# sahaRatul/sela

Hardware: NVIDIA H100
Metric: encode+decode MSamples/s (higher is better)
Workload: dtype f64+int64

## Files before the change

sela_b200/csrc/c_abi.cu:

```cuda
#include <algorithm>
#include <atomic>
#include <cstdarg>
#include <cstdio>
#include <cstdlib>
#include <cstring>
#include <mutex>
#include <thread>
#include <vector>

#include "verify.cuh"

using namespace selab200;

namespace {

thread_local char g_error[512] = "";
std::mutex g_mutex;
std::atomic<uint64_t> g_launches{0};

int fail(int code, const char *fmt, ...)
{
    va_list ap;
    va_start(ap, fmt);
    vsnprintf(g_error, sizeof g_error, fmt, ap);
// ... 180 lines not shown
    if (g_n_ctx == 0)
        return require_ready();
    cudaPointerAttributes attr;
    if (cudaPointerGetAttributes(&attr, device_ptr) != cudaSuccess || attr.type != cudaMemoryTypeDevice) {
        cudaGetLastError();
        return fail(SELAB200_ERR_ARGUMENT, "not a device pointer");
    }
    for (int i = 0; i < g_n_ctx; i++)
        if (g_slots[i].ready && g_slots[i].device == attr.device) {
            tl_ctx = &g_slots[i];
            cudaError_t e = cudaSetDevice(g.device);
            if (e != cudaSuccess)
                return fail(SELAB200_ERR_CUDA, "cudaSetDevice(%d) failed: %s", g.device, cudaGetErrorString(e));
            return 0;
        }
    return fail(SELAB200_ERR_ARGUMENT, "the buffers live on device %d, which the library was not initialised for "
                                       "(selab200_init / selab200_init_devices)", attr.device);
}

size_t align256(size_t v) { return (v + 255) & ~(size_t)255; }

template <typename K>
int set_smem(K kernel, size_t bytes)
{
    static std::mutex m;
    static std::vector<std::pair<std::pair<const void *, int>, size_t>> done;
    int dev = 0;
    CUDA_TRY(cudaGetDevice(&dev));
    const std::pair<const void *, int> key(reinterpret_cast<const void *>(kernel), dev);
    std::lock_guard<std::mutex> lock(m);
    for (auto &e : done)
        if (e.first == key) {
            if (e.second >= bytes)
                return 0;
            CUDA_TRY(cudaFuncSetAttribute(kernel, cudaFuncAttributeMaxDynamicSharedMemorySize, (int)bytes));
            e.second = bytes;
            return 0;
        }
    CUDA_TRY(cudaFuncSetAttribute(kernel, cudaFuncAttributeMaxDynamicSharedMemorySize, (int)bytes));
    done.emplace_back(key, bytes);
    return 0;
}

int launch_check(const char *what)
{
    g_launches.fetch_add(1, std::memory_order_relaxed);
    cudaError_t e = cudaGetLastError();
    if (e != cudaSuccess)
        return fail(SELAB200_ERR_CUDA, "launch of %s failed: %s", what, cudaGetErrorString(e));
    return 0;
}

template <int KIND>
int launch_unit_means(const void *src, size_t n_units, uint32_t channels, double *means, cudaStream_t stream)
{
    const MeanTiling mt = mean_tiling(KIND, channels);
    k_unit_means<KIND><<<(unsigned)((n_units + 31) / 32), 32, unit_means_smem_bytes(mt), stream>>>(src, (uint32_t)n_units,
                                                                                                 channels, means);
    return launch_check("k_unit_means");
}

template <bool STEREO, bool TRACE>
int launch_encode_units(const EncodeParams &p, size_t n_units, selab200_analysis_trace *d_trace, cudaStream_t stream)
{
    constexpr size_t smem = encode_smem_bytes<STEREO>();
    if (int rc = set_smem(k_encode_units<STEREO, TRACE>, smem))
        return rc;
    k_encode_units<STEREO, TRACE><<<(unsigned)n_units, 32, smem, stream>>>(p, d_trace);
    return launch_check("k_encode_units");
}


int encode_device(const int16_t *d_pcm, uint32_t n_frames, uint32_t channels, selab200_subframe_desc *d_descs,
                  uint32_t *d_words, size_t capacity, uint64_t *d_used, int32_t *d_status, void *d_ws,
                  size_t ws_bytes, cudaStream_t stream, bool fresh = true, cudaEvent_t before_scan = nullptr,
                  cudaEvent_t after_scan = nullptr, unsigned long long *h_fill_after = nullptr,
                  uint8_t *d_container = nullptr, unsigned long long sub_base = 0,
                  selab200_analysis_trace *d_trace = nullptr)
{
    if (channels == 0 || channels > SELAB200_MAX_CHANNELS)
        return fail(SELAB200_ERR_ARGUMENT, "channels must be in [1, %d]", SELAB200_MAX_CHANNELS);
    if (ws_bytes < selab200_encode_workspace_bytes(n_frames, channels))
        return fail(SELAB200_ERR_ARGUMENT, "encode workspace too small");
    if (channels == 2 && (reinterpret_cast<uintptr_t>(d_pcm) & 15) != 0)
        return fail(SELAB200_ERR_ARGUMENT, "stereo PCM must be 16-byte aligned on the device");
    if (fresh) {
        CUDA_TRY(cudaMemsetAsync(d_status, 0, sizeof(int32_t), stream));
        CUDA_TRY(cudaMemsetAsync(d_used, 0, sizeof(uint64_t), stream));
    }
    if (n_frames == 0)
        return 0;
    const bool stereo = channels == 2;
    const size_t n_units = encode_units(n_frames, channels);
    const size_t n_sub = (size_t)n_frames * channels;
    EncodeParams p;
    p.pcm = d_pcm;
    p.n_frames = n_frames;
    p.channels = channels;
    p.descs = d_descs;
    p.words = d_words;
    p.capacity = capacity;
    p.words_used = reinterpret_cast<unsigned long long *>(d_used);
    p.status = d_status;
    p.units = static_cast<UnitRecord *>(d_ws);
    p.slots = reinterpret_cast<uint32_t *>(static_cast<char *>(d_ws) + align256(n_units * sizeof(UnitRecord)));
    p.means = reinterpret_cast<double *>(reinterpret_cast<char *>(p.slots) + align256(n_units * (size_t)kSlotWords * 4));
    p.residues = reinterpret_cast<int32_t *>(reinterpret_cast<char *>(p.means) + align256(n_units * sizeof(double)));
    if (int rc = stereo ? launch_unit_means<kMeanStereo>(d_pcm, n_units, channels, p.means, stream)
                        : launch_unit_means<kMeanPcm>(d_pcm, n_units, channels, p.means, stream))
        return rc;
    const int rc_units = stereo ? (d_trace ? launch_encode_units<true, true>(p, n_units, d_trace, stream)
                                           : launch_encode_units<true, false>(p, n_units, nullptr, stream))
                                : (d_trace ? launch_encode_units<false, true>(p, n_units, d_trace, stream)
                                           : launch_encode_units<false, false>(p, n_units, nullptr, stream));
    if (rc_units)
        return rc_units;
    const unsigned scan_ctas = (unsigned)((n_sub + kScanTile - 1) / kScanTile);
    k_encode_sizes<<<scan_ctas, kScanTile, 0, stream>>>(p);
    if (int rc = launch_check("k_encode_sizes"))
        return rc;
    if (before_scan)
        CUDA_TRY(cudaStreamWaitEvent(stream, before_scan, 0));
    k_encode_scan<<<scan_ctas, kScanTile, 0, stream>>>(p);
    if (int rc = launch_check("k_encode_scan"))
        return rc;
    CUDA_TRY(cudaMemcpyAsync(d_used, p.residues, 8, cudaMemcpyDeviceToDevice, stream));
    if (h_fill_after)
        CUDA_TRY(cudaMemcpyAsync(h_fill_after, d_used, 8, cudaMemcpyDeviceToHost, stream));
    if (after_scan)
        CUDA_TRY(cudaEventRecord(after_scan, stream));
    if (d_container) {
        k_encode_gather_container<<<(unsigned)((n_sub + 7) / 8), 256, 0, stream>>>(p, d_container, sub_base);
        return launch_check("k_encode_gather_container");
    }
    k_encode_gather<<<(unsigned)((n_sub + 7) / 8), 256, 0, stream>>>(p);
    return launch_check("k_encode_gather");
}

int launch_rice_decode(const DecodeParams &p, int which, cudaStream_t stream)
{
    const size_t n_sub = (size_t)p.n_frames * p.channels;
    const unsigned blocks = (unsigned)((n_sub + 32 * kRiceWarps - 1) / (32 * kRiceWarps));
    k_rice_decode<kRiceRing, kRiceBatch><<<blocks, 32 * kRiceWarps, 0, stream>>>(p, which);
    return launch_check(which ? "k_rice_decode(res)" : "k_rice_decode(refl)");
}

int rice_split_log2(size_t n_sub)
{
    if (const char *env = std::getenv("SELAB200_RICE_SPLIT")) {
        const long v = std::atol(env);
        if (v <= 0)
            return -1;
        int l = 0;
        while ((1 << (l + 1)) <= v && l < 4)
            l++;
        return l;
    }
    const size_t sms = (size_t)g.sms;
    if (n_sub >= 81 * sms)
        return 0;
    int l = 0;
    while (l < 4 && (n_sub << l) < 270 * sms)
// ... 322 lines not shown
            char keep[sizeof g_error];
            memcpy(keep, g_error, sizeof keep);
            g_n_ctx = i + 1;
            shutdown_all();
            memcpy(g_error, keep, sizeof keep);
            return rc;
        }
    }
    g_n_ctx = count;
    tl_ctx = &g_slots[0];
    CUDA_TRY(cudaSetDevice(g_slots[0].device));
    return 0;
}

int selab200_init(int device) { return selab200_init_devices(1, &device); }

int selab200_device_count(void)
{
    std::lock_guard<std::mutex> lock(g_mutex);
    return g_n_ctx;
}

void selab200_shutdown(void)
{
    std::lock_guard<std::mutex> lock(g_mutex);
    shutdown_all();
}

void *selab200_host_alloc(size_t bytes)
{
    void *p = nullptr;
    if (cudaMallocHost(&p, bytes ? bytes : 1) != cudaSuccess) {
        fail(SELAB200_ERR_CUDA, "cudaMallocHost(%zu) failed", bytes);
        return nullptr;
    }
    return p;
}

void selab200_host_free(void *p)
{
    if (p)
        cudaFreeHost(p);
}

size_t selab200_encode_words_bound(uint32_t n_frames, uint32_t channels)
{
    return (size_t)n_frames * channels * kSlotWords + 64;
}

size_t selab200_encode_workspace_bytes(uint32_t n_frames, uint32_t channels)
{
    const size_t n_units = encode_units(n_frames, channels);
    return align256(n_units * sizeof(UnitRecord)) + align256(n_units * (size_t)kSlotWords * 4) +
           align256(n_units * sizeof(double)) + n_units * (size_t)kFrame * 4 + 256;
}

size_t selab200_decode_workspace_bytes(uint32_t n_frames, uint32_t channels)
{
    const size_t n_sub = (size_t)n_frames * channels;
    return align256(n_sub * 128 * 4) + align256(n_sub * kFrame * 4) + align256(synthesis_warps(n_sub) * 32 * 4) +
           align256(n_sub * 64) + 256;
}

size_t selab200_verify_workspace_bytes(uint32_t n_frames, uint32_t channels)
{
    return align256(selab200_decode_workspace_bytes(n_frames, channels)) + align256((size_t)n_frames * channels * kFrame * 2);
}

int selab200_encode_frames_device(const int16_t *d_pcm, uint32_t n_frames, uint32_t channels,
                                  selab200_subframe_desc *d_descs, uint32_t *d_words, size_t words_capacity,
                                  uint64_t *d_words_used, int32_t *d_status, void *d_workspace,
                                  size_t workspace_bytes, void *stream)
{
    std::lock_guard<std::mutex> lock(g_mutex);
    if (int rc = d_pcm ? require_ready_for(d_pcm) : require_ready())
        return rc;
    if (!d_pcm || !d_descs || !d_words || !d_words_used || !d_status || !d_workspace)
        return fail(SELAB200_ERR_ARGUMENT, "null device pointer");
    return encode_device(d_pcm, n_frames, channels, d_descs, d_words, words_capacity, d_words_used, d_status,
                         d_workspace, workspace_bytes, (cudaStream_t)stream);
}

int selab200_decode_frames_device(const selab200_subframe_desc *d_descs, uint32_t n_frames, uint32_t channels,
                                  const uint32_t *d_words, size_t n_words, int16_t *d_pcm_out, int32_t *d_status,
                                  void *d_workspace, size_t workspace_bytes, void *stream)
{
    std::lock_guard<std::mutex> lock(g_mutex);
    if (int rc = d_descs ? require_ready_for(d_descs) : require_ready())
        return rc;
    if (!d_descs || !d_words || !d_pcm_out || !d_status || !d_workspace)
        return fail(SELAB200_ERR_ARGUMENT, "null device pointer");
    return decode_device(d_descs, n_frames, channels, d_words, n_words, d_pcm_out, d_status, d_workspace,
                         workspace_bytes, (cudaStream_t)stream);
}

int selab200_verify_frames_device(const selab200_subframe_desc *d_descs, uint32_t n_frames, uint32_t channels,
                                  const uint32_t *d_words, size_t n_words, const int16_t *d_pcm_ref,
                                  selab200_verify_entry *d_entries, uint64_t *d_n_differing, int32_t *d_status,
                                  void *d_workspace, size_t workspace_bytes, void *stream)
{
    std::lock_guard<std::mutex> lock(g_mutex);
    if (int rc = d_descs ? require_ready_for(d_descs) : require_ready())
        return rc;
    if (!d_descs || !d_words || !d_pcm_ref || !d_entries || !d_n_differing || !d_status || !d_workspace)
        return fail(SELAB200_ERR_ARGUMENT, "null device pointer");
    return verify_device(d_descs, n_frames, channels, d_words, n_words, d_pcm_ref, d_entries,
                         reinterpret_cast<unsigned long long *>(d_n_differing), d_status, d_workspace, workspace_bytes,
// ... 1001 lines not shown
}

int selab200_fir_probe(const int32_t *samples, const int32_t *orders, const int64_t *c, uint32_t n, int wide,
                       int32_t *residues)
{
    std::lock_guard<std::mutex> lock(g_mutex);
    if (int rc = require_ready())
        return rc;
    if (!samples || !orders || !c || !residues)
        return fail(SELAB200_ERR_ARGUMENT, "null pointer");
    if (n == 0)
        return 0;
    const int hi = wide ? 65535 : 32767, lo = wide ? -65535 : -32768;
    for (size_t i = 0; i < (size_t)n * kFrame; i++)
        if (samples[i] > hi || samples[i] < lo)
            return fail(SELAB200_ERR_RANGE, "sample %zu = %d outside the domain of the row form", i, samples[i]);
    for (uint32_t i = 0; i < n; i++)
        if (orders[i] < 0 || orders[i] > kMaxOrder)
            return fail(SELAB200_ERR_RANGE, "order %d of signal %u outside 0..%d", orders[i], i, kMaxOrder);
    const size_t sig = (size_t)n * kFrame * 4, cb = (size_t)n * (kMaxOrder + 1) * 8;
    if (int rc = g.in.ensure(sig)) return rc;
    if (int rc = g.work.ensure(sig)) return rc;
    if (int rc = g.aux.ensure(cb + (size_t)n * 4)) return rc;
    long long *d_c = static_cast<long long *>(g.aux.ptr);
    int32_t *d_orders = reinterpret_cast<int32_t *>(d_c + (size_t)n * (kMaxOrder + 1));
    CUDA_TRY(cudaMemcpyAsync(g.in.ptr, samples, sig, cudaMemcpyHostToDevice, g.stream));
    CUDA_TRY(cudaMemcpyAsync(d_c, c, cb, cudaMemcpyHostToDevice, g.stream));
    CUDA_TRY(cudaMemcpyAsync(d_orders, orders, (size_t)n * 4, cudaMemcpyHostToDevice, g.stream));
    k_fir_probe<<<n, 32, 0, g.stream>>>(static_cast<const int32_t *>(g.in.ptr), d_orders, d_c, wide,
                                        static_cast<int32_t *>(g.work.ptr));
    if (int rc = launch_check("k_fir_probe"))
        return rc;
    CUDA_TRY(cudaMemcpyAsync(residues, g.work.ptr, sig, cudaMemcpyDeviceToHost, g.stream));
    CUDA_TRY(cudaStreamSynchronize(g.stream));
    return 0;
}


int selab200_lpc_residues(const int32_t *samples, uint32_t n_sub, uint8_t *order, int32_t *q, int32_t *residues)
{
    std::lock_guard<std::mutex> lock(g_mutex);
    if (int rc = require_ready())
        return rc;
    if (!samples || !order || !q || !residues)
        return fail(SELAB200_ERR_ARGUMENT, "null pointer");
    if (n_sub == 0)
        return 0;
    for (size_t i = 0; i < (size_t)n_sub * kFrame; i++)
        if (samples[i] > 65535 || samples[i] < -65535)
            return fail(SELAB200_ERR_RANGE, "sample %zu = %d outside the 17-bit domain of 16-bit audio", i, samples[i]);
    const size_t sig = (size_t)n_sub * kFrame * 4;
    if (int rc = g.in.ensure(sig)) return rc;
    if (int rc = g.work.ensure(sig)) return rc;
    if (int rc = g.aux.ensure(align256((size_t)n_sub * sizeof(double)) + (size_t)n_sub * kMaxOrder * 4 + n_sub + 256)) return rc;
    double *d_means = static_cast<double *>(g.aux.ptr);
    int32_t *d_q = reinterpret_cast<int32_t *>(static_cast<char *>(g.aux.ptr) + align256((size_t)n_sub * sizeof(double)));
    uint8_t *d_order = reinterpret_cast<uint8_t *>(d_q + (size_t)n_sub * kMaxOrder);
    CUDA_TRY(cudaMemcpyAsync(g.in.ptr, samples, sig, cudaMemcpyHostToDevice, g.stream));
    if (int rc = launch_unit_means<kMeanPlanar>(g.in.ptr, n_sub, 1, d_means, g.stream))
        return rc;
    k_lpc_residues<<<n_sub, 32, 0, g.stream>>>(static_cast<const int32_t *>(g.in.ptr), d_means, n_sub, d_order, d_q,
                                               static_cast<int32_t *>(g.work.ptr));
    if (int rc = launch_check("k_lpc_residues"))
        return rc;
    CUDA_TRY(cudaMemcpyAsync(residues, g.work.ptr, sig, cudaMemcpyDeviceToHost, g.stream));
    CUDA_TRY(cudaMemcpyAsync(q, d_q, (size_t)n_sub * kMaxOrder * 4, cudaMemcpyDeviceToHost, g.stream));
    CUDA_TRY(cudaMemcpyAsync(order, d_order, n_sub, cudaMemcpyDeviceToHost, g.stream));
    CUDA_TRY(cudaStreamSynchronize(g.stream));
    return 0;
}

int selab200_lpc_samples(const int32_t *residues, uint32_t n_sub, const uint8_t *order, const int32_t *q,
                         int32_t *samples)
{
    std::lock_guard<std::mutex> lock(g_mutex);
    if (int rc = require_ready())
        return rc;
    if (!residues || !order || !q || !samples)
        return fail(SELAB200_ERR_ARGUMENT, "null pointer");
    if (n_sub == 0)
        return 0;
    for (uint32_t i = 0; i < n_sub; i++)
        if (order[i] > kMaxOrder)
            return fail(SELAB200_ERR_BITSTREAM, "order[%u] = %u exceeds %d", i, order[i], kMaxOrder);
    const size_t sig = (size_t)n_sub * kFrame * 4;
    if (int rc = g.in.ensure(sig)) return rc;
    if (int rc = g.work.ensure(sig)) return rc;
    if (int rc = g.aux.ensure((size_t)n_sub * kMaxOrder * 4 + n_sub + 256)) return rc;
    int32_t *d_q = static_cast<int32_t *>(g.aux.ptr);
    uint8_t *d_order = reinterpret_cast<uint8_t *>(d_q + (size_t)n_sub * kMaxOrder);
    CUDA_TRY(cudaMemcpyAsync(g.in.ptr, residues, sig, cudaMemcpyHostToDevice, g.stream));
    CUDA_TRY(cudaMemcpyAsync(d_q, q, (size_t)n_sub * kMaxOrder * 4, cudaMemcpyHostToDevice, g.stream));
    CUDA_TRY(cudaMemcpyAsync(d_order, order, n_sub, cudaMemcpyHostToDevice, g.stream));
    k_lpc_samples<<<n_sub, 32, 0, g.stream>>>(static_cast<const int32_t *>(g.in.ptr), n_sub, d_order, d_q,
                                              static_cast<int32_t *>(g.work.ptr));
    if (int rc = launch_check("k_lpc_samples"))
        return rc;
    CUDA_TRY(cudaMemcpyAsync(samples, g.work.ptr, sig, cudaMemcpyDeviceToHost, g.stream));
    CUDA_TRY(cudaStreamSynchronize(g.stream));
    return 0;
}

int selab200_rice_encode(const int32_t *values, const uint32_t *counts, uint32_t n_streams, uint32_t stride,
                         uint32_t *rice_param, uint32_t *n_words, uint32_t *words, uint32_t words_stride)
{
    std::lock_guard<std::mutex> lock(g_mutex);
    if (int rc = require_ready())
        return rc;
    if (!values || !counts || !rice_param || !n_words || !words)
        return fail(SELAB200_ERR_ARGUMENT, "null pointer");
    if (stride > (uint32_t)kFrame)
        return fail(SELAB200_ERR_ARGUMENT, "stride %u exceeds %d values per stream", stride, kFrame);
    for (uint32_t i = 0; i < n_streams; i++)
        if (counts[i] > stride)
// ... 61 lines not shown
```

sela_b200/csrc/kernels.cuh:

```cuda
#pragma once

#include "lpc.cuh"
#include "rice.cuh"
#include "rice_vs.cuh"

namespace selab200 {

enum { kMeanPcm = 0, kMeanStereo = 1, kMeanPlanar = 2 };
constexpr int kMeanTile = 64;
constexpr int kMeanSlots = 16;

struct MeanTiling {
    uint32_t units_per_row;
    uint32_t step;
    uint32_t row_stride;
    uint32_t rows_max;
    uint32_t row_words;
};

__host__ __device__ inline MeanTiling mean_tiling(int kind, uint32_t channels)
{
    MeanTiling t;
    uint32_t span = 1;
    if (kind == kMeanPcm) {
        t.units_per_row = channels;
        t.step = 2 * channels;
        t.row_stride = (uint32_t)kFrame * 2 * channels;
        t.rows_max = 31 / channels + 2 < 32 ? 31 / channels + 2 : 32;
        span = (2 * channels + 5) / 4;
    } else {
        t.units_per_row = kind == kMeanStereo ? 3 : 1;
        t.step = 4;
        t.row_stride = (uint32_t)kFrame * 4;
        t.rows_max = kind == kMeanStereo ? 12 : 32;
    }
    const uint32_t d = span | 1u;
    const uint32_t need = kMeanTile * t.step / 4 + 4;
    t.row_words = need + ((d - need) & 31u);
    return t;
}

template <int KIND>
__global__ void __launch_bounds__(32) k_unit_means(const void *src, uint32_t n_units, uint32_t channels, double *means)
{
    extern __shared__ __align__(16) uint32_t staged[];
    const MeanTiling mt = mean_tiling(KIND, channels);
    const int lane = lane_id();
    const uint32_t u0 = blockIdx.x * 32, u = u0 + lane;
    const uint32_t u_last = u0 + 31 < n_units ? u0 + 31 : n_units - 1;
    const uint32_t first = u0 / mt.units_per_row, n_rows = u_last / mt.units_per_row - first + 1;
    const uint32_t mine = u < n_units ? u : u_last;
    const uint32_t row = mine / mt.units_per_row - first, role = mine % mt.units_per_row;

    const char *base = static_cast<const char *>(src) + (size_t)first * mt.row_stride;
    const uint32_t mis = (uint32_t)reinterpret_cast<uintptr_t>(base) & 15u;
    const uint4 *pieces = reinterpret_cast<const uint4 *>(base - mis);
    const uint32_t tile_pieces = kMeanTile * mt.step / 16;
    const uint32_t per_row = (mis + kMeanTile * mt.step + 15) / 16, total = n_rows * per_row;
    uint32_t goff[kMeanSlots], soff[kMeanSlots];
#pragma unroll
    for (int s = 0; s < kMeanSlots; s++) {
        const uint32_t v = lane + 32 * s, r = v / per_row, k = v - r * per_row;
        goff[s] = r * (mt.row_stride / 16) + k;
        soff[s] = r * mt.row_words + 4 * k;
    }
    uint4 buf[kMeanSlots];
    auto fetch = [&](int t) {
#pragma unroll
        for (int s = 0; s < kMeanSlots; s++)
            if (lane + 32 * s < total)
                buf[s] = pieces[goff[s] + t * tile_pieces];
    };
    const char *at = reinterpret_cast<const char *>(staged) + row * mt.row_words * 4 + mis + (KIND == kMeanPcm ? 2 * role : 0);

    MeanChain chain;
    fetch(0);
    for (int t = 0; t < kFrame / kMeanTile; t++) {
        __syncwarp();
#pragma unroll
        for (int s = 0; s < kMeanSlots; s++)
            if (lane + 32 * s < total) {
                staged[soff[s]] = buf[s].x;
                staged[soff[s] + 1] = buf[s].y;
                staged[soff[s] + 2] = buf[s].z;
                staged[soff[s] + 3] = buf[s].w;
            }
        __syncwarp();
        if (t + 1 < kFrame / kMeanTile)
            fetch(t + 1);
#pragma unroll 8
        for (int j = 0; j < kMeanTile; j++) {
            int x;
            if (KIND == kMeanPcm) {
                x = *reinterpret_cast<const int16_t *>(at + j * mt.step);
            } else if (KIND == kMeanStereo) {
                const uint32_t pair = *reinterpret_cast<const uint32_t *>(at + 4 * j);
                const int a = (int)(pair << 16) >> 16, b = (int)pair >> 16;
                x = role == 0 ? a : role == 1 ? b : a - b;
            } else {
                x = *reinterpret_cast<const int32_t *>(at + 4 * j);
            }
            chain.add(x);
        }
    }
    if (u < n_units)
        means[u] = chain.mean();
}

inline size_t unit_means_smem_bytes(const MeanTiling &mt) { return (size_t)mt.rows_max * mt.row_words * 4; }


constexpr uint32_t kSlotWords = 1600;
constexpr uint32_t kSlotReflWords = 32;

struct __align__(16) UnitRecord {
    uint32_t order;
    uint32_t refl_k, refl_words;
    uint32_t res_k, res_words;
    uint32_t flags;
    uint32_t pad[2];
};

struct EncodeParams {
    const int16_t *pcm;
    uint32_t n_frames, channels;
    selab200_subframe_desc *descs;
    uint32_t *words;
    unsigned long long capacity;
    unsigned long long *words_used;
    int32_t *status;
    UnitRecord *units;
    uint32_t *slots;
    double *means;
    int32_t *residues;
};

__host__ __device__ inline uint32_t encode_units(uint32_t n_frames, uint32_t channels)
{
    return channels == 2 ? n_frames * 3u : n_frames * channels;
}

template <bool STEREO, bool TRACE = false>
__global__ void __launch_bounds__(32) k_encode_units(EncodeParams p, selab200_analysis_trace *trace)
{
    constexpr int kRow = kHistoryPad + kFrame;
    constexpr int kLoWords = (kHistoryPad + kFrame) / 32;
    extern __shared__ __align__(16) unsigned char smem_raw[];
    int16_t *s16 = reinterpret_cast<int16_t *>(smem_raw);
    uint32_t *lo_bits = reinterpret_cast<uint32_t *>(smem_raw + kRow * 2);
    constexpr size_t kSigBytes = kRow * 2 + (STEREO ? kLoWords * 4 : 0);
    AnalysisScratch &scratch = *reinterpret_cast<AnalysisScratch *>(smem_raw + kSigBytes);
    static_assert(kCoefAlias + sizeof(CoefSmem) <= sizeof(AnalysisScratch) && kCoefAlias % 16 == 0, "predictor alias");
    CoefSmem &cf = *reinterpret_cast<CoefSmem *>(smem_raw + kSigBytes + kCoefAlias);

    const int lane = lane_id();
    const uint32_t unit = blockIdx.x;
    const uint32_t frame = STEREO ? unit / 3 : unit / p.channels;
    const uint32_t role = STEREO ? unit % 3 : unit % p.channels;

    const int16_t *src = p.pcm + (size_t)frame * kFrame * p.channels;
    for (int j = lane; j < kHistoryPad / 2; j += 32)
        reinterpret_cast<uint32_t *>(s16)[j] = 0;
    int16_t *row = s16 + kHistoryPad;
    Signal sig;
    sig.a = row;
    sig.lo = nullptr;
    if (STEREO) {
        const uint4 *src128 = reinterpret_cast<const uint4 *>(src);
        if (role < 2) {
            const uint32_t sel = role ? 0x7632 : 0x5410;
            for (int j = lane; j < kFrame / 4; j += 32) {
                const uint4 v = src128[j];
                reinterpret_cast<uint2 *>(row)[j] = make_uint2(__byte_perm(v.x, v.y, sel), __byte_perm(v.z, v.w, sel));
            }
        } else {
            if (lane < kHistoryPad / 32)
                lo_bits[lane] = 0;
            uint32_t *lo = lo_bits + kHistoryPad / 32;
            for (int it = 0; it < kFrame / 128; it++) {
                const uint4 v = src128[it * 32 + lane];
                const uint32_t pr[4] = {v.x, v.y, v.z, v.w};
                int d[4];
#pragma unroll
                for (int e = 0; e < 4; e++)
                    d[e] = ((int)(pr[e] << 16) >> 16) - ((int)pr[e] >> 16);
                const uint32_t h01 = ((uint32_t)(d[0] >> 1) & 0xffffu) | ((uint32_t)(d[1] >> 1) << 16);
                const uint32_t h23 = ((uint32_t)(d[2] >> 1) & 0xffffu) | ((uint32_t)(d[3] >> 1) << 16);
                reinterpret_cast<uint2 *>(row)[it * 32 + lane] = make_uint2(h01, h23);
                uint32_t nib = (d[0] & 1) | ((d[1] & 1) << 1) | ((d[2] & 1) << 2) | ((d[3] & 1) << 3);
                nib <<= 4 * (lane & 7);
                nib |= __shfl_xor_sync(kFull, nib, 1);
                nib |= __shfl_xor_sync(kFull, nib, 2);
                nib |= __shfl_xor_sync(kFull, nib, 4);
                if ((lane & 7) == 0)
                    lo[it * 4 + (lane >> 3)] = nib;
            }
            sig.lo = lo;
        }
    } else {
        for (int j = lane; j < kFrame; j += 32)
            row[j] = src[(size_t)j * p.channels + role];
    }
    __syncwarp();

    int32_t *res = p.residues + (size_t)unit * kFrame;
    warp_autocorrelation(sig, scratch, shfl_d(lane == 0 ? p.means[unit] : 0.0, 0));
    if constexpr (TRACE) {
        selab200_analysis_trace &tr = trace[unit];
        if (lane == 0)
            tr.mean = p.means[unit];
        for (int i = lane; i <= kMaxOrder; i += 32)
            tr.ac[i] = scratch.ac[i];
    }
    warp_schur(scratch);
    const int order = warp_order_and_quantise(scratch, cf);
    warp_coefficients(cf, scratch.t(), order);
    if constexpr (TRACE) {
        selab200_analysis_trace &tr = trace[unit];
        for (int i = lane; i < kMaxOrder; i += 32) {
            tr.k[i] = scratch.kk()[i];
            tr.q[i] = cf.q[i];
        }
        for (int i = lane; i <= kMaxOrder; i += 32)
            tr.c[i] = i == 0 ? 0 : coef_at(cf, i);
        if (lane == 0)
            tr.order = order;
    }
    static_assert(kPlaneBytes <= kCoefAlias, "FIR digit planes");
    uint32_t *planes = reinterpret_cast<uint32_t *>(scratch.ring);
    if (STEREO && role == 2)
        warp_fir_residual<true>(sig, cf, order, planes, res);
    else
        warp_fir_residual<false>(sig, cf, order, planes, res);

    const RiceChoice cq = warp_rice_choose(cf.q, order);
    const RiceChoice cr = warp_rice_choose(res, kFrame);
    const bool too_large = cq.words > kSlotReflWords || cr.words > kSlotWords - kSlotReflWords;
    uint32_t *slot = p.slots + (size_t)unit * kSlotWords;
    if (!too_large) {
        warp_rice_pack(cf.q, order, cq, slot);
        warp_rice_pack(res, kFrame, cr, slot + kSlotReflWords);
    }
    __syncwarp();
    for (int l = lane; l < kFrame * 4 / 128; l += 32)
        asm volatile("discard.global.L2 [%0], 128;" ::"l"(res + l * 32) : "memory");
    if (lane == 0) {
        UnitRecord u;
        u.order = order;
        u.refl_k = cq.k;
        u.refl_words = cq.words;
        u.res_k = cr.k;
        u.res_words = cr.words;
        u.flags = too_large ? 1u : 0u;
        u.pad[0] = u.pad[1] = 0;
        p.units[unit] = u;
    }
}

template <bool STEREO>
constexpr size_t encode_smem_bytes()
{
    return (size_t)(kHistoryPad + kFrame) * 2 + (STEREO ? (kHistoryPad + kFrame) / 8 : 0) + sizeof(AnalysisScratch);
}
// ... 534 lines not shown
    int32_t *row = p.ws_res + (size_t)sub * kFrame;
    if (k == 0) {
        sm.row_res[seg] = row;
        sm.row_out[seg] = diff ? static_cast<void *>(row) : static_cast<void *>(out + mine.channel);
        sm.row_mode[seg] = !proc ? 0 : diff ? 2 : 1;
    }
    __syncwarp();
    segment_synthesis(sm, start, k, n, seg, n_seg, proc ? mine.lpc_order : 0, p.ws_q + (size_t)sub * 128, ch);

    if (exists && !frame_ok) {
        for (int t = k; t < kFrame; t += n)
            out[(size_t)t * ch + pos] = 0;
    }
}

__global__ void __launch_bounds__(128) k_diff_fixup(DecodeParams p)
{
    const uint32_t frame = blockIdx.x, ch = p.channels;
    const selab200_subframe_desc *fd = p.descs + (size_t)frame * ch;
    bool any = false;
    for (uint32_t pos = 0; pos < ch; pos++)
        any |= fd[pos].subframe_type == 1;
    if (!any || !frame_check(fd, ch, p.n_words))
        return;
    int16_t *out = p.pcm_out + (size_t)frame * kFrame * ch;
    for (uint32_t pos = 0; pos < ch; pos++) {
        const selab200_subframe_desc d = fd[pos];
        if (d.subframe_type != 1)
            continue;
        const int32_t *diff = p.ws_res + ((size_t)frame * ch + pos) * kFrame;
        for (int t = threadIdx.x; t < kFrame; t += blockDim.x)
            out[(size_t)t * ch + d.channel] =
                (int16_t)(uint16_t)((uint32_t)out[(size_t)t * ch + d.parent_channel] - (uint32_t)diff[t]);
    }
}


struct Row17 {
    __align__(16) int16_t a[kHistoryPad + kFrame];
    uint32_t lo[(kHistoryPad + kFrame) / 32];
    __device__ __forceinline__ Signal stage(const int32_t *src)
    {
        const int lane = lane_id();
        for (int i = lane; i < kHistoryPad / 2; i += 32)
            reinterpret_cast<uint32_t *>(a)[i] = 0;
        if (lane < kHistoryPad / 32)
            lo[lane] = 0;
        stage_17bit_row(src, a + kHistoryPad, lo + kHistoryPad / 32);
        __syncwarp();
        return Signal{a + kHistoryPad, lo + kHistoryPad / 32};
    }
};

__global__ void __launch_bounds__(32) k_lpc_residues(const int32_t *samples, const double *means, uint32_t n_sub,
                                                     uint8_t *order_out, int32_t *q_out, int32_t *residues)
{
    __shared__ __align__(16) AnalysisScratch scratch;
    __shared__ __align__(16) CoefSmem cf;
    __shared__ __align__(16) Row17 row;
    const uint32_t sub = blockIdx.x;
    const int lane = lane_id();
    const Signal sig = row.stage(samples + (size_t)sub * kFrame);
    warp_autocorrelation(sig, scratch, means[sub]);
    warp_schur(scratch);
    const int order = warp_order_and_quantise(scratch, cf);
    warp_coefficients(cf, scratch.t(), order);
    warp_fir_residual<true>(sig, cf, order, reinterpret_cast<uint32_t *>(scratch.ring), residues + (size_t)sub * kFrame);
    for (int i = lane; i < kMaxOrder; i += 32)
        q_out[(size_t)sub * kMaxOrder + i] = i < order ? cf.q[i] : 0;
    if (lane == 0)
        order_out[sub] = (uint8_t)order;
}

__global__ void __launch_bounds__(32) k_fir_probe(const int32_t *samples, const int32_t *orders, const long long *c,
                                                  int wide, int32_t *residues)
{
    __shared__ __align__(16) AnalysisScratch scratch;
    __shared__ __align__(16) CoefSmem cf;
    __shared__ __align__(16) Row17 row;
    const uint32_t sub = blockIdx.x;
    const int lane = lane_id();
    const int32_t *src = samples + (size_t)sub * kFrame;
    Signal sig = row.stage(src);
    if (!wide) {
        for (int j = lane; j < kFrame; j += 32)
            row.a[kHistoryPad + j] = (int16_t)src[j];
        sig.lo = nullptr;
    }
    const int order = orders[sub];
    for (int i = lane; i < 112; i += 32) {
        const long long v = i < order ? c[(size_t)sub * (kMaxOrder + 1) + i + 1] : 0;
        cf.clo[i] = (uint32_t)v;
        cf.chi[i] = (int32_t)(v >> 32);
    }
    __syncwarp();
    uint32_t *planes = reinterpret_cast<uint32_t *>(scratch.ring);
    int32_t *res = residues + (size_t)sub * kFrame;
    if (wide)
        warp_fir_residual<true>(sig, cf, order, planes, res);
    else
        warp_fir_residual<false>(sig, cf, order, planes, res);
}

__global__ void __launch_bounds__(32) k_lpc_samples(const int32_t *residues, uint32_t n_sub, const uint8_t *order_in,
                                                    const int32_t *q_in, int32_t *samples)
{
    __shared__ __align__(16) SegSmem sm;
    const uint32_t sub = blockIdx.x;
    const int lane = lane_id();
    const int order = min((int)order_in[sub], kMaxOrder);
    const int n = segment_width(order);
    if (lane == 0) {
        sm.row_res[0] = residues + (size_t)sub * kFrame;
        sm.row_out[0] = samples + (size_t)sub * kFrame;
        sm.row_mode[0] = 2;
    }
// ... 73 lines not shown
```

sela_b200/csrc/lpc.cuh:

```cuda
#pragma once

#include "common.cuh"
#include "lpc_tables.cuh"

namespace selab200 {

struct CoefSmem {
    uint32_t clo[112];
    int32_t  chi[112];
    int32_t  q[104];
};
struct AnalysisScratch {
    double ring[256];
    double ac[128];
    __device__ __forceinline__ double *kk() { return ring; }
    __device__ __forceinline__ double *t() { return ring + 104; }
};
using LpcSmem = AnalysisScratch;
constexpr size_t kCoefAlias = 208 * sizeof(double);

__device__ __forceinline__ long long coef_at(const CoefSmem &cf, int j)
{
    return (long long)(((unsigned long long)(uint32_t)cf.chi[j - 1] << 32) | cf.clo[j - 1]);
}

__device__ __forceinline__ int ring_chunk(int chunk)
{
    chunk &= 127;
    return chunk ^ ((chunk >> 3) & 1);
}
__device__ __forceinline__ int ring_index(int p)
{
    return (ring_chunk(p >> 1) << 1) | (p & 1);
}

__device__ __forceinline__ double sample_to_x(int s)
{
    const double rcp = 1.0 / 32767.0;
    const double a = (double)s;
    const double q0 = __dmul_rn(a, rcp);
    const double r = __fma_rn(-q0, 32767.0, a);
    return __fma_rn(r, rcp, q0);
}
__device__ __forceinline__ double sample_to_x_div(int s) { return ddiv((double)s, 32767.0); }

struct MeanChain {
    double sum = 0.0;
    __device__ __forceinline__ void add(int s) { sum = dadd(sum, sample_to_x(s)); }
    __device__ __forceinline__ double mean() const { return ddiv(sum, (double)kFrame); }
};

template <typename Sig>
__device__ void warp_autocorrelation(const Sig &sig, LpcSmem &sm, const double mean)
{
    const int lane = lane_id();

    {
        double2 *r2 = reinterpret_cast<double2 *>(sm.ring);
        r2[64 + lane] = make_double2(0.0, 0.0);
        r2[96 + lane] = make_double2(0.0, 0.0);
    }
    double acc0 = 0.0, acc1 = 0.0, acc2 = 0.0, acc3 = 0.0;
    double p1 = 0.0, p2 = 0.0, p3 = 0.0;
    const char *ringb = reinterpret_cast<const char *>(sm.ring);
    int own_off[8];
#pragma unroll
    for (int i = 0; i < 8; i++) {
        const int rel = i - lane;
        own_off[i] = 16 * (2 * rel + ((rel >> 2) & 1));
    }

    for (int tile = 0; tile < kFrame / 128; tile++) {
        __syncwarp();
#pragma unroll
        for (int r = 0; r < 4; r++) {
            int j = tile * 128 + r * 32 + lane;
            sm.ring[ring_index(j)] = dsub(sample_to_x(sig.at(j)), mean);
        }
        __syncwarp();
        for (int blk = 0; blk < 4; blk++) {
            const int gb = (tile * 32 + blk * 8) * 32;
            const char *bbase = ringb + (gb & 2047);
#pragma unroll
            for (int i = 0; i < 8; i++) {
                const int oo = (gb + own_off[i]) & 2047;
                const double2 o0 = *reinterpret_cast<const double2 *>(ringb + oo);
                const double2 o1 = *reinterpret_cast<const double2 *>(ringb + (oo ^ 16));
                constexpr int kSw[8] = {0, 0, 0, 0, 16, 16, 16, 16};
                const double2 b0 = *reinterpret_cast<const double2 *>(bbase + ((32 * i) ^ kSw[i]));
                const double2 b1 = *reinterpret_cast<const double2 *>(bbase + ((32 * i + 16) ^ kSw[i]));
                const double c0 = o0.x, c1 = o0.y, c2 = o1.x, c3 = o1.y;
                acc0 = dadd(acc0, dmul(b0.x, c0));
                acc1 = dadd(acc1, dmul(b0.x, p1));
                acc2 = dadd(acc2, dmul(b0.x, p2));
                acc3 = dadd(acc3, dmul(b0.x, p3));
                acc0 = dadd(acc0, dmul(b0.y, c1));
                acc1 = dadd(acc1, dmul(b0.y, c0));
                acc2 = dadd(acc2, dmul(b0.y, p1));
                acc3 = dadd(acc3, dmul(b0.y, p2));
                acc0 = dadd(acc0, dmul(b1.x, c2));
                acc1 = dadd(acc1, dmul(b1.x, c1));
                acc2 = dadd(acc2, dmul(b1.x, c0));
                acc3 = dadd(acc3, dmul(b1.x, p1));
                acc0 = dadd(acc0, dmul(b1.y, c3));
                acc1 = dadd(acc1, dmul(b1.y, c2));
                acc2 = dadd(acc2, dmul(b1.y, c1));
                acc3 = dadd(acc3, dmul(b1.y, c0));
                p1 = c3;
                p2 = c2;
                p3 = c1;
            }
        }
    }
    __syncwarp();
    sm.ac[4 * lane + 0] = acc0;
    sm.ac[4 * lane + 1] = acc1;
    sm.ac[4 * lane + 2] = acc2;
    sm.ac[4 * lane + 3] = acc3;
    __syncwarp();
    const double ac0 = sm.ac[0];
    __syncwarp();
#pragma unroll
    for (int t = 0; t < 4; t++) {
        int i = lane + 32 * t;
        if (i >= 1 && i <= kMaxOrder)
            sm.ac[i] = ddiv(sm.ac[i], ac0);
    }
    if (lane == 0)
        sm.ac[0] = 1.0;
    __syncwarp();
}

__device__ void warp_schur(LpcSmem &sm)
{
    const int lane = lane_id();
    double *kk = sm.kk();
    double g0[4], g1[4];
#pragma unroll
    for (int m = 0; m < 4; m++) {
        int j = 4 * lane + m;
        double v = (j < kMaxOrder) ? sm.ac[j + 1] : 0.0;
        g0[m] = v;
        g1[m] = v;
    }
    double err = sm.ac[0];
    double head = shfl_d(g1[0], 0);
    double k = ddiv(-head, err);
    err = dadd(err, dmul(head, k));
    if (lane == 0)
        kk[0] = k;
    for (int i = 1; i < kMaxOrder; i++) {
        const double kp = k;
        const double nxt = shfl_down_d(g1[0], 1);
        double up[4] = {g1[1], g1[2], g1[3], nxt};
#pragma unroll
        for (int m = 0; m < 4; m++) {
            double n1 = dadd(up[m], dmul(kp, g0[m]));
            double n0 = dadd(dmul(up[m], kp), g0[m]);
            g1[m] = n1;
            g0[m] = n0;
        }
        head = shfl_d(g1[0], 0);
        k = ddiv(-head, err);
        err = dadd(err, dmul(head, k));
        if (lane == 0)
            kk[i] = k;
    }
    __syncwarp();
}


__device__ __forceinline__ bool reflection_significant(double kv) { return fabs(kv) > 0.05; }

__device__ __forceinline__ int quantise_reflection(int i, double kv)
{
    const double sqrt2 = 1.4142135623730950488016887242096;
    double v;
    if (i == 0)
        v = floor(dmul(64.0, dadd(-1.0, dmul(sqrt2, dsqrt(dadd(kv, 1.0))))));
    else if (i == 1)
        v = floor(dmul(64.0, dadd(-1.0, dmul(sqrt2, dsqrt(dadd(-kv, 1.0))))));
    else
        v = floor(dmul(64.0, kv));
    return isnan(v) ? 0 : __double2int_rz(v);
}

__device__ int warp_order_and_quantise(LpcSmem &sm, CoefSmem &cf)
{
    const int lane = lane_id();
    const double *kk = sm.kk();
    int best = -1;
#pragma unroll
    for (int t = 0; t < 4; t++) {
        int i = lane + 32 * t;
        if (i < kMaxOrder && reflection_significant(kk[i]))
            best = i;
    }
    best = __reduce_max_sync(kFull, best);
    const int order = best < 0 ? 1 : best + 1;

#pragma unroll
    for (int t = 0; t < 4; t++) {
        int i = lane + 32 * t;
        if (i < order) {
            cf.q[i] = quantise_reflection(i, kk[i]);
        } else if (i < 104) {
            cf.q[i] = 0;
        }
    }
    __syncwarp();
    return order;
}

// ... 368 lines not shown
```

Measured before the change: 12450.

## Compute high-lag autocorrelation tails in mean kernel and trim per-lane lag work

The unit-means kernel now keeps three staged tiles and makes a second pass that computes the mean plus the highest autocorrelation lags (from lag 96 upward), storing several stats per unit. The per-unit autocorrelation then computes only three lags per lane over a simpler unswizzled ring with a 96-sample history, and the Schur recursion is relaid out lane-strided so that finished lag slots are skipped. The intent is to move part of the FP64 multiply-add work off the serialized per-warp encode kernel and to shrink its inner loop. In exchange the means kernel does more work and uses more shared memory, the workspace grows, and the integer-to-double conversion now uses a bit trick.

```diff
diff --git a/sela_b200/csrc/c_abi.cu b/sela_b200/csrc/c_abi.cu
--- a/sela_b200/csrc/c_abi.cu
+++ b/sela_b200/csrc/c_abi.cu
@@ -256,11 +256,11 @@
 }
 
 template <int KIND>
-int launch_unit_means(const void *src, size_t n_units, uint32_t channels, double *means, cudaStream_t stream)
+int launch_unit_means(const void *src, size_t n_units, uint32_t channels, double *stats, cudaStream_t stream)
 {
     const MeanTiling mt = mean_tiling(KIND, channels);
     k_unit_means<KIND><<<(unsigned)((n_units + 31) / 32), 32, unit_means_smem_bytes(mt), stream>>>(src, (uint32_t)n_units,
-                                                                                                 channels, means);
+                                                                                                 channels, stats);
     return launch_check("k_unit_means");
 }
 
@@ -308,10 +308,10 @@
     p.status = d_status;
     p.units = static_cast<UnitRecord *>(d_ws);
     p.slots = reinterpret_cast<uint32_t *>(static_cast<char *>(d_ws) + align256(n_units * sizeof(UnitRecord)));
-    p.means = reinterpret_cast<double *>(reinterpret_cast<char *>(p.slots) + align256(n_units * (size_t)kSlotWords * 4));
-    p.residues = reinterpret_cast<int32_t *>(reinterpret_cast<char *>(p.means) + align256(n_units * sizeof(double)));
-    if (int rc = stereo ? launch_unit_means<kMeanStereo>(d_pcm, n_units, channels, p.means, stream)
-                        : launch_unit_means<kMeanPcm>(d_pcm, n_units, channels, p.means, stream))
+    p.stats = reinterpret_cast<double *>(reinterpret_cast<char *>(p.slots) + align256(n_units * (size_t)kSlotWords * 4));
+    p.residues = reinterpret_cast<int32_t *>(reinterpret_cast<char *>(p.stats) + align256(n_units * kUnitStats * sizeof(double)));
+    if (int rc = stereo ? launch_unit_means<kMeanStereo>(d_pcm, n_units, channels, p.stats, stream)
+                        : launch_unit_means<kMeanPcm>(d_pcm, n_units, channels, p.stats, stream))
         return rc;
     const int rc_units = stereo ? (d_trace ? launch_encode_units<true, true>(p, n_units, d_trace, stream)
                                            : launch_encode_units<true, false>(p, n_units, nullptr, stream))
@@ -740,7 +740,7 @@
 {
     const size_t n_units = encode_units(n_frames, channels);
     return align256(n_units * sizeof(UnitRecord)) + align256(n_units * (size_t)kSlotWords * 4) +
-           align256(n_units * sizeof(double)) + n_units * (size_t)kFrame * 4 + 256;
+           align256(n_units * kUnitStats * sizeof(double)) + n_units * (size_t)kFrame * 4 + 256;
 }
 
 size_t selab200_decode_workspace_bytes(uint32_t n_frames, uint32_t channels)
@@ -1848,14 +1848,15 @@
     const size_t sig = (size_t)n_sub * kFrame * 4;
     if (int rc = g.in.ensure(sig)) return rc;
     if (int rc = g.work.ensure(sig)) return rc;
-    if (int rc = g.aux.ensure(align256((size_t)n_sub * sizeof(double)) + (size_t)n_sub * kMaxOrder * 4 + n_sub + 256)) return rc;
-    double *d_means = static_cast<double *>(g.aux.ptr);
-    int32_t *d_q = reinterpret_cast<int32_t *>(static_cast<char *>(g.aux.ptr) + align256((size_t)n_sub * sizeof(double)));
+    const size_t stats_bytes = align256((size_t)n_sub * kUnitStats * sizeof(double));
+    if (int rc = g.aux.ensure(stats_bytes + (size_t)n_sub * kMaxOrder * 4 + n_sub + 256)) return rc;
+    double *d_stats = static_cast<double *>(g.aux.ptr);
+    int32_t *d_q = reinterpret_cast<int32_t *>(static_cast<char *>(g.aux.ptr) + stats_bytes);
     uint8_t *d_order = reinterpret_cast<uint8_t *>(d_q + (size_t)n_sub * kMaxOrder);
     CUDA_TRY(cudaMemcpyAsync(g.in.ptr, samples, sig, cudaMemcpyHostToDevice, g.stream));
-    if (int rc = launch_unit_means<kMeanPlanar>(g.in.ptr, n_sub, 1, d_means, g.stream))
-        return rc;
-    k_lpc_residues<<<n_sub, 32, 0, g.stream>>>(static_cast<const int32_t *>(g.in.ptr), d_means, n_sub, d_order, d_q,
+    if (int rc = launch_unit_means<kMeanPlanar>(g.in.ptr, n_sub, 1, d_stats, g.stream))
+        return rc;
+    k_lpc_residues<<<n_sub, 32, 0, g.stream>>>(static_cast<const int32_t *>(g.in.ptr), d_stats, n_sub, d_order, d_q,
                                                static_cast<int32_t *>(g.work.ptr));
     if (int rc = launch_check("k_lpc_residues"))
         return rc;
diff --git a/sela_b200/csrc/kernels.cuh b/sela_b200/csrc/kernels.cuh
--- a/sela_b200/csrc/kernels.cuh
+++ b/sela_b200/csrc/kernels.cuh
@@ -8,7 +8,11 @@
 
 enum { kMeanPcm = 0, kMeanStereo = 1, kMeanPlanar = 2 };
 constexpr int kMeanTile = 64;
+constexpr int kMeanTiles = kFrame / kMeanTile;
+constexpr int kMeanStaged = 3;
 constexpr int kMeanSlots = 16;
+static_assert(kTailLag0 == 3 * kMeanTile / 2, "the second walk reads d[j - 96] from the tile two (first half of j's "
+                                               "tile) or one (second half) before");
 
 struct MeanTiling {
     uint32_t units_per_row;
@@ -41,7 +45,7 @@
 }
 
 template <int KIND>
-__global__ void __launch_bounds__(32) k_unit_means(const void *src, uint32_t n_units, uint32_t channels, double *means)
+__global__ void __launch_bounds__(32) k_unit_means(const void *src, uint32_t n_units, uint32_t channels, double *stats)
 {
     extern __shared__ __align__(16) uint32_t staged[];
     const MeanTiling mt = mean_tiling(KIND, channels);
@@ -71,43 +75,84 @@
             if (lane + 32 * s < total)
                 buf[s] = pieces[goff[s] + t * tile_pieces];
     };
+    const uint32_t tile_bytes = mt.rows_max * mt.row_words * 4;
     const char *at = reinterpret_cast<const char *>(staged) + row * mt.row_words * 4 + mis + (KIND == kMeanPcm ? 2 * role : 0);
+    auto tile_at = [&](int t) { return at + (t % kMeanStaged) * tile_bytes; };
+    auto sample = [&](const char *p, int j) {
+        if (KIND == kMeanPcm)
+            return (int)*reinterpret_cast<const int16_t *>(p + j * mt.step);
+        if (KIND == kMeanStereo) {
+            const uint32_t pair = *reinterpret_cast<const uint32_t *>(p + 4 * j);
+            const int a = (int)(pair << 16) >> 16, b = (int)pair >> 16;
+            return role == 0 ? a : role == 1 ? b : a - b;
+        }
+        return *reinterpret_cast<const int32_t *>(p + 4 * j);
+    };
+    auto land = [&](int t, int next) {
+        __syncwarp();
+        uint32_t *slot = staged + (t % kMeanStaged) * (tile_bytes / 4);
+#pragma unroll
+        for (int s = 0; s < kMeanSlots; s++)
+            if (lane + 32 * s < total) {
+                slot[soff[s]] = buf[s].x;
+                slot[soff[s] + 1] = buf[s].y;
+                slot[soff[s] + 2] = buf[s].z;
+                slot[soff[s] + 3] = buf[s].w;
+            }
+        __syncwarp();
+        if (next >= 0)
+            fetch(next);
+    };
 
     MeanChain chain;
     fetch(0);
-    for (int t = 0; t < kFrame / kMeanTile; t++) {
-        __syncwarp();
-#pragma unroll
-        for (int s = 0; s < kMeanSlots; s++)
-            if (lane + 32 * s < total) {
-                staged[soff[s]] = buf[s].x;
-                staged[soff[s] + 1] = buf[s].y;
-                staged[soff[s] + 2] = buf[s].z;
-                staged[soff[s] + 3] = buf[s].w;
+    for (int t = 0; t < kMeanTiles; t++) {
+        land(t, t + 1 < kMeanTiles ? t + 1 : 0);
+        const char *p = tile_at(t);
+#pragma unroll 8
+        for (int j = 0; j < kMeanTile; j++)
+            chain.add(sample(p, j));
+    }
+    const double mean = chain.mean();
+
+    double tail0 = 0.0, tail1 = 0.0, tail2 = 0.0, tail3 = 0.0, tail4 = 0.0;
+    double w1 = 0.0, w2 = 0.0, w3 = 0.0, w4 = 0.0;
+    for (int t = 0; t < kMeanTiles; t++) {
+        land(t, t + 1 < kMeanTiles ? t + 1 : -1);
+#pragma unroll
+        for (int h = 0; h < 2; h++) {
+            if (t * kMeanTile + h * (kMeanTile / 2) < kTailLag0)
+                continue;
+            const char *p = tile_at(t);
+            const char *q = tile_at(t + h + kMeanStaged - 2);
+#pragma unroll 8
+            for (int i = 0; i < kMeanTile / 2; i++) {
+                const double d = centred(sample(p, h * (kMeanTile / 2) + i), mean);
+                const double w0 = centred(sample(q, (1 - h) * (kMeanTile / 2) + i), mean);
+                tail0 = dadd(tail0, dmul(d, w0));
+                tail1 = dadd(tail1, dmul(d, w1));
+                tail2 = dadd(tail2, dmul(d, w2));
+                tail3 = dadd(tail3, dmul(d, w3));
+                tail4 = dadd(tail4, dmul(d, w4));
+                w4 = w3;
+                w3 = w2;
+                w2 = w1;
+                w1 = w0;
             }
-        __syncwarp();
-        if (t + 1 < kFrame / kMeanTile)
-            fetch(t + 1);
-#pragma unroll 8
-        for (int j = 0; j < kMeanTile; j++) {
-            int x;
-            if (KIND == kMeanPcm) {
-                x = *reinterpret_cast<const int16_t *>(at + j * mt.step);
-            } else if (KIND == kMeanStereo) {
-                const uint32_t pair = *reinterpret_cast<const uint32_t *>(at + 4 * j);
-                const int a = (int)(pair << 16) >> 16, b = (int)pair >> 16;
-                x = role == 0 ? a : role == 1 ? b : a - b;
-            } else {
-                x = *reinterpret_cast<const int32_t *>(at + 4 * j);
-            }
-            chain.add(x);
-        }
-    }
-    if (u < n_units)
-        means[u] = chain.mean();
-}
-
-inline size_t unit_means_smem_bytes(const MeanTiling &mt) { return (size_t)mt.rows_max * mt.row_words * 4; }
+        }
+    }
+    if (u < n_units) {
+        double *out = stats + (size_t)kUnitStats * u;
+        out[0] = mean;
+        out[1] = tail0;
+        out[2] = tail1;
+        out[3] = tail2;
+        out[4] = tail3;
+        out[5] = tail4;
+    }
+}
+
+inline size_t unit_means_smem_bytes(const MeanTiling &mt) { return (size_t)kMeanStaged * mt.rows_max * mt.row_words * 4; }
 
 
 constexpr uint32_t kSlotWords = 1600;
@@ -131,7 +176,7 @@
     int32_t *status;
     UnitRecord *units;
     uint32_t *slots;
-    double *means;
+    double *stats;
     int32_t *residues;
 };
 
@@ -204,11 +249,11 @@
     __syncwarp();
 
     int32_t *res = p.residues + (size_t)unit * kFrame;
-    warp_autocorrelation(sig, scratch, shfl_d(lane == 0 ? p.means[unit] : 0.0, 0));
+    warp_autocorrelation(sig, scratch, lane < kUnitStats ? p.stats[(size_t)kUnitStats * unit + lane] : 0.0);
     if constexpr (TRACE) {
         selab200_analysis_trace &tr = trace[unit];
         if (lane == 0)
-            tr.mean = p.means[unit];
+            tr.mean = p.stats[(size_t)kUnitStats * unit];
         for (int i = lane; i <= kMaxOrder; i += 32)
             tr.ac[i] = scratch.ac[i];
     }
@@ -849,7 +894,7 @@
     }
 };
 
-__global__ void __launch_bounds__(32) k_lpc_residues(const int32_t *samples, const double *means, uint32_t n_sub,
+__global__ void __launch_bounds__(32) k_lpc_residues(const int32_t *samples, const double *stats, uint32_t n_sub,
                                                      uint8_t *order_out, int32_t *q_out, int32_t *residues)
 {
     __shared__ __align__(16) AnalysisScratch scratch;
@@ -858,7 +903,7 @@
     const uint32_t sub = blockIdx.x;
     const int lane = lane_id();
     const Signal sig = row.stage(samples + (size_t)sub * kFrame);
-    warp_autocorrelation(sig, scratch, means[sub]);
+    warp_autocorrelation(sig, scratch, lane < kUnitStats ? stats[(size_t)kUnitStats * sub + lane] : 0.0);
     warp_schur(scratch);
     const int order = warp_order_and_quantise(scratch, cf);
     warp_coefficients(cf, scratch.t(), order);
diff --git a/sela_b200/csrc/lpc.cuh b/sela_b200/csrc/lpc.cuh
--- a/sela_b200/csrc/lpc.cuh
+++ b/sela_b200/csrc/lpc.cuh
@@ -24,20 +24,10 @@
     return (long long)(((unsigned long long)(uint32_t)cf.chi[j - 1] << 32) | cf.clo[j - 1]);
 }
 
-__device__ __forceinline__ int ring_chunk(int chunk)
-{
-    chunk &= 127;
-    return chunk ^ ((chunk >> 3) & 1);
-}
-__device__ __forceinline__ int ring_index(int p)
-{
-    return (ring_chunk(p >> 1) << 1) | (p & 1);
-}
-
 __device__ __forceinline__ double sample_to_x(int s)
 {
     const double rcp = 1.0 / 32767.0;
-    const double a = (double)s;
+    const double a = __dsub_rn(__hiloint2double(0x43300000, (int)((unsigned)s ^ 0x80000000u)), 4503601774854144.0);
     const double q0 = __dmul_rn(a, rcp);
     const double r = __fma_rn(-q0, 32767.0, a);
     return __fma_rn(r, rcp, q0);
@@ -50,73 +40,57 @@
     __device__ __forceinline__ double mean() const { return ddiv(sum, (double)kFrame); }
 };
 
+__device__ __forceinline__ double centred(int s, double mean) { return dsub(sample_to_x(s), mean); }
+
+constexpr int kTailLag0 = 96;
+constexpr int kUnitStats = 1 + kMaxOrder + 1 - kTailLag0;
+
+constexpr int kRingHistory = 96;
+constexpr int kRingTile = 128;
 template <typename Sig>
-__device__ void warp_autocorrelation(const Sig &sig, LpcSmem &sm, const double mean)
-{
-    const int lane = lane_id();
-
-    {
-        double2 *r2 = reinterpret_cast<double2 *>(sm.ring);
-        r2[64 + lane] = make_double2(0.0, 0.0);
-        r2[96 + lane] = make_double2(0.0, 0.0);
-    }
-    double acc0 = 0.0, acc1 = 0.0, acc2 = 0.0, acc3 = 0.0;
-    double p1 = 0.0, p2 = 0.0, p3 = 0.0;
-    const char *ringb = reinterpret_cast<const char *>(sm.ring);
-    int own_off[8];
-#pragma unroll
-    for (int i = 0; i < 8; i++) {
-        const int rel = i - lane;
-        own_off[i] = 16 * (2 * rel + ((rel >> 2) & 1));
-    }
-
-    for (int tile = 0; tile < kFrame / 128; tile++) {
+__device__ void warp_autocorrelation(const Sig &sig, LpcSmem &sm, const double stat)
+{
+    const int lane = lane_id();
+    const double mean = shfl_d(stat, 0);
+    if (lane >= 1 && lane <= kMaxOrder + 1 - kTailLag0)
+        sm.ac[kTailLag0 - 1 + lane] = stat;
+
+    double acc0 = 0.0, acc1 = 0.0, acc2 = 0.0;
+    double m1 = 0.0, m2 = 0.0;
+    const double *own = sm.ring + kRingHistory - 3 * lane;
+    for (int tile = 0; tile < kFrame / kRingTile; tile++) {
         __syncwarp();
 #pragma unroll
-        for (int r = 0; r < 4; r++) {
-            int j = tile * 128 + r * 32 + lane;
-            sm.ring[ring_index(j)] = dsub(sample_to_x(sig.at(j)), mean);
-        }
+        for (int r = 0; r < 3; r++)
+            sm.ring[32 * r + lane] = tile ? sm.ring[kRingHistory + 32 * (r + 1) + lane] : 0.0;
+#pragma unroll
+        for (int r = 0; r < 4; r++)
+            sm.ring[kRingHistory + 32 * r + lane] = centred(sig.at(tile * kRingTile + 32 * r + lane), mean);
         __syncwarp();
-        for (int blk = 0; blk < 4; blk++) {
-            const int gb = (tile * 32 + blk * 8) * 32;
-            const char *bbase = ringb + (gb & 2047);
-#pragma unroll
-            for (int i = 0; i < 8; i++) {
-                const int oo = (gb + own_off[i]) & 2047;
-                const double2 o0 = *reinterpret_cast<const double2 *>(ringb + oo);
-                const double2 o1 = *reinterpret_cast<const double2 *>(ringb + (oo ^ 16));
-                constexpr int kSw[8] = {0, 0, 0, 0, 16, 16, 16, 16};
-                const double2 b0 = *reinterpret_cast<const double2 *>(bbase + ((32 * i) ^ kSw[i]));
-                const double2 b1 = *reinterpret_cast<const double2 *>(bbase + ((32 * i + 16) ^ kSw[i]));
-                const double c0 = o0.x, c1 = o0.y, c2 = o1.x, c3 = o1.y;
-                acc0 = dadd(acc0, dmul(b0.x, c0));
-                acc1 = dadd(acc1, dmul(b0.x, p1));
-                acc2 = dadd(acc2, dmul(b0.x, p2));
-                acc3 = dadd(acc3, dmul(b0.x, p3));
-                acc0 = dadd(acc0, dmul(b0.y, c1));
-                acc1 = dadd(acc1, dmul(b0.y, c0));
-                acc2 = dadd(acc2, dmul(b0.y, p1));
-                acc3 = dadd(acc3, dmul(b0.y, p2));
-                acc0 = dadd(acc0, dmul(b1.x, c2));
-                acc1 = dadd(acc1, dmul(b1.x, c1));
-                acc2 = dadd(acc2, dmul(b1.x, c0));
-                acc3 = dadd(acc3, dmul(b1.x, p1));
-                acc0 = dadd(acc0, dmul(b1.y, c3));
-                acc1 = dadd(acc1, dmul(b1.y, c2));
-                acc2 = dadd(acc2, dmul(b1.y, c1));
-                acc3 = dadd(acc3, dmul(b1.y, c0));
-                p1 = c3;
-                p2 = c2;
-                p3 = c1;
-            }
-        }
-    }
-    __syncwarp();
-    sm.ac[4 * lane + 0] = acc0;
-    sm.ac[4 * lane + 1] = acc1;
-    sm.ac[4 * lane + 2] = acc2;
-    sm.ac[4 * lane + 3] = acc3;
+#pragma unroll 8
+        for (int g = 0; g < kRingTile / 4; g++) {
+            const double2 b0 = *reinterpret_cast<const double2 *>(sm.ring + kRingHistory + 4 * g);
+            const double2 b1 = *reinterpret_cast<const double2 *>(sm.ring + kRingHistory + 4 * g + 2);
+            const double c0 = own[4 * g], c1 = own[4 * g + 1], c2 = own[4 * g + 2], c3 = own[4 * g + 3];
+            acc0 = dadd(acc0, dmul(b0.x, c0));
+            acc1 = dadd(acc1, dmul(b0.x, m1));
+            acc2 = dadd(acc2, dmul(b0.x, m2));
+            acc0 = dadd(acc0, dmul(b0.y, c1));
+            acc1 = dadd(acc1, dmul(b0.y, c0));
+            acc2 = dadd(acc2, dmul(b0.y, m1));
+            acc0 = dadd(acc0, dmul(b1.x, c2));
+            acc1 = dadd(acc1, dmul(b1.x, c1));
+            acc2 = dadd(acc2, dmul(b1.x, c0));
+            acc0 = dadd(acc0, dmul(b1.y, c3));
+            acc1 = dadd(acc1, dmul(b1.y, c2));
+            acc2 = dadd(acc2, dmul(b1.y, c1));
+            m1 = c3;
+            m2 = c2;
+        }
+    }
+    sm.ac[3 * lane + 0] = acc0;
+    sm.ac[3 * lane + 1] = acc1;
+    sm.ac[3 * lane + 2] = acc2;
     __syncwarp();
     const double ac0 = sm.ac[0];
     __syncwarp();
@@ -138,7 +112,7 @@
     double g0[4], g1[4];
 #pragma unroll
     for (int m = 0; m < 4; m++) {
-        int j = 4 * lane + m;
+        int j = lane + 32 * m;
         double v = (j < kMaxOrder) ? sm.ac[j + 1] : 0.0;
         g0[m] = v;
         g1[m] = v;
@@ -149,16 +123,22 @@
     err = dadd(err, dmul(head, k));
     if (lane == 0)
         kk[0] = k;
+    const int next = (lane + 1) & 31;
     for (int i = 1; i < kMaxOrder; i++) {
         const double kp = k;
-        const double nxt = shfl_down_d(g1[0], 1);
-        double up[4] = {g1[1], g1[2], g1[3], nxt};
+        double up[4];
+#pragma unroll
+        for (int m = 0; m < 4; m++)
+            if (32 * m < kMaxOrder - i)
+                up[m] = shfl_d(lane == 0 ? (m < 3 ? g1[m + 1] : 0.0) : g1[m], next);
 #pragma unroll
         for (int m = 0; m < 4; m++) {
-            double n1 = dadd(up[m], dmul(kp, g0[m]));
-            double n0 = dadd(dmul(up[m], kp), g0[m]);
-            g1[m] = n1;
-            g0[m] = n0;
+            if (32 * m < kMaxOrder - i) {
+                double n1 = dadd(up[m], dmul(kp, g0[m]));
+                double n0 = dadd(dmul(up[m], kp), g0[m]);
+                g1[m] = n1;
+                g0[m] = n0;
+            }
         }
         head = shfl_d(g1[0], 0);
         k = ddiv(-head, err);
```

Result: no change. 12550 (median of 6 runs) (+0.8%).
